# CrystalSixone/VLN-MAGIC

Measured on AMD Instinct MI355X. Metric: trajectory-steps/sec (whole node), MAGIC-S R2R pretrain, higher is better.
Workload: dtype bf16

## Files before the change

include/magic_hip.h:

```cpp
#ifndef MAGIC_HIP_H
#define MAGIC_HIP_H
#ifdef __cplusplus
extern "C" {
#endif

#define MAGIC_OK 0
#define MAGIC_ERR_ARG (-1)
#define MAGIC_ERR_LAUNCH (-2)
#define MAGIC_ERR_UNSUPPORTED (-3)

int magic_abi_version(void);
int magic_build_id(char* out, int len);
int magic_device_info(int* cu_count, int* clock_khz, char* arch, int arch_len);

int magic_gemm(int dtype, int layout, int batch, int nh, int M, int N, int K,
               const void* A, int lda, long long sAb, long long sAh,
               const void* B, int ldb, long long sBb, long long sBh,
               void* C, int ldc, long long sCb, long long sCh, int c_f32, int accumulate,
               const float* bias, int epilogue, const void* aux, int ldaux,
               const void* residual, int ldr, void* C2, int ldc2,
               float alpha, int splitk, float* bias_grad, void* stream);
int magic_gemm_set_big(int mode);
#define MAGIC_GEMM_FORM_PLAIN 0x1
#define MAGIC_GEMM_FORM_XCD 0x2
// ... 209 lines not shown
int magic_sap_fuse_bwd(int B, int K, int Vp, const float* g_raw, const float* l_raw, const float* fuse_raw,
                       const unsigned char* gmask, const unsigned char* lmask, const int* fsrc, const unsigned char* bwmask,
                       int use_gate, const float* dgl, const float* dll, const float* dfl,
                       float* dg_raw, float* dl_raw, float* dfuse_raw, void* stream);

int magic_step_rng(unsigned long long base_seed, unsigned* counter, float rw_temp, int* seed_out, float* rw_out, float* zero_me,
                   float* scale_state, float growth, float backoff, int interval, void* stream);
int magic_seed_scale(const float* scale_dev);
int magic_loss_assemble(const float* rows, int n_rows, const float* row_w, float row_scale, const float* kd_rows, int n_kd,
                        float* slots, const float* rw, float alpha, int has_kd, float* out, void* stream);

int magic_rowgate_fwd(int dtype, int M, int H, int mode, const void* x, const void* e, const float* wx, const float* we,
                      const float* b0, const float* b1, float* out_s, void* out, float* gsave, void* stream);
int magic_rowgate_bwd(int dtype, int M, int H, int mode, const void* x, const void* e, const float* wx, const float* we, const float* gsave,
                      const float* dy, const void* dout, void* dx, void* de, float* dwx, float* dwe, float* db0, float* db1, void* stream);

int magic_sumsq(long long n, const float* g, float* out, void* stream);
int magic_adamw(long long n, float* p, float* g, float* m, float* v, void* shadow, int shadow_dtype,
                float lr, float b1, float b2, float eps, float wd, float step_size,
                const float* sumsq, float max_norm, float gscale, const float* lr_ss, long long n_decay, int zero_grad,
                unsigned* overflow, float* scale_state, int* sched_step, int decay_first, void* stream);
int magic_sumsq_sched(long long n, const float* g, float* out, int* step, float lr0, int warmup, int total, float b1, float b2,
                      float* lr_ss, void* stream);
int magic_sched_step(int* step, float lr0, int warmup, int total, float b1, float b2, float* lr_ss, float* zero_me, void* stream);
int magic_cast(int dtype16, int to16, long long n, const void* x, void* y, void* stream);
int magic_add_n(int dtype, long long n, int count, const void* const* xs, void* y, void* stream);
int magic_add(int dtype, long long n, const void* x, void* y, void* stream);
int magic_dact(int dtype, int kind, long long n, const void* dy, const void* z, void* dz, void* stream);

int magic_view_gather(int dtype, int Np, int V, int D, const void* table, int n_viewpoints, const int* vp_row,
                      const int* order, void* out, void* stream);

int magic_set_f32_mfma(int mode);
int magic_get_f32_mfma(void);

typedef struct {
  const void* Wqkv; const float* bqkv; const void* Wo; const float* bo; const float* g1; const float* be1;
  const void* W1; const float* bi; const void* W2; const float* bo2; const float* g2; const float* be2;
  void *qkv, *P, *Pd, *ctx, *a, *z, *g, *out; float *rstd_a, *rstd_o;
  unsigned site_attn, site_ao, site_out, pad_;
} magic_enc_layer;
typedef struct { const void* x; const unsigned char* kmask; int nsamp, N, ldp, nlayers; magic_enc_layer L[6]; } magic_enc_seg;
typedef struct { magic_enc_seg seg[2]; int nseg; float p_attn, p_hidden, eps, scale; const unsigned* seed;
                 unsigned* sync; int sync_words, pad2_; } magic_enc_params;
int magic_encoder_supported(int dtype, int H, int I, int nh, int N, int nlayers);
int magic_encoder_params_bytes(void);
// ... 72 lines not shown
```

vln-magic_amd/csrc/optim.hip:

```cpp
#include "common.hpp"
#include "group.hpp"

struct SchedArgs { int* step; float lr0; int warmup, total; float b1, b2; float* lr_ss; };
__device__ __forceinline__ void sched_advance(const SchedArgs& a) {
  const int gs = a.step[0];
  a.step[0] = gs + 1;
  const int t = a.step[1] + 1;
  a.step[1] = t;
  double f = gs < a.warmup ? (double)gs / (double)a.warmup : fmax(0.0, (double)(a.total - gs) / (double)(a.total - a.warmup));
  double lr = (double)a.lr0 * f;
  if (lr <= 0.0) lr = 1e-8;
  const double ss = lr * sqrt(1.0 - pow((double)a.b2, (double)t)) / (1.0 - pow((double)a.b1, (double)t));
  a.lr_ss[0] = (float)lr; a.lr_ss[1] = (float)ss;
}
__global__ __launch_bounds__(1024) void sumsq_kernel(long long n, const float* __restrict__ g, float* out, SchedArgs sa) {
  __shared__ float red[16];
  if (sa.step && blockIdx.x == 0 && threadIdx.x == 0) sched_advance(sa);
  float s = 0.f;
  const long long n4 = n >> 2, stride = (long long)gridDim.x * 1024;
  for (long long i = (long long)blockIdx.x * 1024 + threadIdx.x; i < n4; i += 4 * stride) {
    float4 v[4];
#pragma unroll
    for (int u = 0; u < 4; ++u) v[u] = (i + u * stride < n4) ? ((const float4*)g)[i + u * stride] : make_float4(0.f, 0.f, 0.f, 0.f);
#pragma unroll
// ... 26 lines not shown
    if (zero_g)
      for (long long i = (long long)blockIdx.x * 256 + threadIdx.x; i < n; i += (long long)gridDim.x * 256) g[i] = 0.f;
    return;
  }
  if (sumsq && max_norm > 0.f) {
    const float nrm = sqrtf(sumsq[0]) * gscale;
    clip = gscale * fminf(1.f, max_norm / (nrm + 1e-6f));
  }
  for (long long i = (long long)blockIdx.x * 256 + threadIdx.x; i < n; i += (long long)gridDim.x * 256) {
    const float gi = g[i] * clip;
    const float mi = b1 * m[i] + (1.f - b1) * gi;
    const float vi = b2 * v[i] + (1.f - b2) * gi * gi;
    float pi = p[i];
    const bool dec = wd > 0.f && i < n_decay;
    if (dec && decay_first) pi -= lr * wd * pi;
    pi -= step_size * mi / (sqrtf(vi) + eps);
    if (dec && !decay_first) pi -= lr * wd * pi;
    m[i] = mi; v[i] = vi; p[i] = pi;
    if (shadow) shadow[i] = (Hh)pi;
    if (zero_g) g[i] = 0.f;
  }
}

template <typename Hh>
__global__ __launch_bounds__(256) void cast_f32_h16_kernel(long long n, const float* x, Hh* y) {
  const long long n4 = n >> 2;
  for (long long i = (long long)blockIdx.x * 256 + threadIdx.x; i < n4; i += (long long)gridDim.x * 256) {
    const float4 v = ((const float4*)x)[i];
    h16x4<Hh> o; o[0] = (Hh)v.x; o[1] = (Hh)v.y; o[2] = (Hh)v.z; o[3] = (Hh)v.w;
    ((h16x4<Hh>*)y)[i] = o;
  }
  if (blockIdx.x == 0 && threadIdx.x < (n & 3)) y[(n4 << 2) + threadIdx.x] = (Hh)x[(n4 << 2) + threadIdx.x];
}

template <typename Hh>
__global__ __launch_bounds__(256) void cast_h16_f32_kernel(long long n, const Hh* x, float* y) {
  for (long long i = (long long)blockIdx.x * 256 + threadIdx.x; i < n; i += (long long)gridDim.x * 256) y[i] = (float)x[i];
}

template <typename T>
__global__ __launch_bounds__(256) void add_kernel(long long n, const T* x, T* y) {
  for (long long i = (long long)blockIdx.x * 256 + threadIdx.x; i < n; i += (long long)gridDim.x * 256) y[i] = from_f<T>(to_f(y[i]) + to_f(x[i]));
}

struct AddN { const void* x[8]; int n; };
template <typename T>
// ... 34 lines not shown
  return launch_status();
}
extern "C" int magic_sumsq_sched(long long n, const float* g, float* out, int* step, float lr0, int warmup, int total, float b1, float b2,
                                 float* lr_ss, void* stream) {
  if (n <= 0 || ((uintptr_t)g & 15) || !step || !lr_ss || warmup <= 0 || total <= warmup) return MAGIC_ERR_ARG;
  const int nb = nblocks(n, 4096);
  hipLaunchKernelGGL(sumsq_kernel, dim3(nb > 256 ? 256 : nb), dim3(1024), 0, (hipStream_t)stream, n, g, out, SchedArgs{step, lr0, warmup, total, b1, b2, lr_ss});
  return launch_status();
}

extern "C" int magic_adamw(long long n, float* p, float* g, float* m, float* v, void* shadow, int shadow_dtype,
                           float lr, float b1, float b2, float eps, float wd, float step_size,
                           const float* sumsq, float max_norm, float gscale, const float* lr_ss, long long n_decay, int zero_grad,
                           unsigned* overflow, float* scale_state, int* sched_step, int decay_first, void* stream) {
  if (n <= 0 || (shadow && !dtype_is16(shadow_dtype))) return MAGIC_ERR_ARG;
  if (scale_state && !sumsq) return MAGIC_ERR_ARG;
  if (n_decay < 0) n_decay = n;
  if (shadow && shadow_dtype == DT_F16)
    hipLaunchKernelGGL(adamw_kernel<f16>, dim3(nblocks(n, 256)), dim3(256), 0, (hipStream_t)stream, n, p, g, m, v, (f16*)shadow, lr, b1, b2, eps, wd,
                       step_size, sumsq, max_norm, gscale, lr_ss, n_decay, zero_grad, overflow, scale_state, sched_step, decay_first);
  else
    hipLaunchKernelGGL(adamw_kernel<bf16>, dim3(nblocks(n, 256)), dim3(256), 0, (hipStream_t)stream, n, p, g, m, v, (bf16*)shadow, lr, b1, b2, eps, wd,
                       step_size, sumsq, max_norm, gscale, lr_ss, n_decay, zero_grad, overflow, scale_state, sched_step, decay_first);
  return launch_status();
}

extern "C" int magic_cast(int dtype16, int to16, long long n, const void* x, void* y, void* stream) {
  if (n <= 0 || !dtype_is16(dtype16)) return MAGIC_ERR_ARG;
  const hipStream_t st = (hipStream_t)stream;
  if (to16) {
    if (((uintptr_t)x & 15) || ((uintptr_t)y & 7)) return MAGIC_ERR_ARG;
    DISPATCH_H(dtype16, hipLaunchKernelGGL(cast_f32_h16_kernel<TY>, dim3(nblocks(n, 1024)), dim3(256), 0, st, n, (const float*)x, (TY*)y));
  } else {
    DISPATCH_H(dtype16, hipLaunchKernelGGL(cast_h16_f32_kernel<TY>, dim3(nblocks(n, 256)), dim3(256), 0, st, n, (const TY*)x, (float*)y));
  }
  return launch_status();
}

extern "C" int magic_add(int dtype, long long n, const void* x, void* y, void* stream) {
  if (n <= 0) return MAGIC_ERR_ARG;
  DISPATCH_T(dtype, hipLaunchKernelGGL(add_kernel<TY>, dim3(nblocks(n, 256)), dim3(256), 0, (hipStream_t)stream, n, (const TY*)x, (TY*)y));
  return launch_status();
}

extern "C" int magic_add_n(int dtype, long long n, int count, const void* const* xs, void* y, void* stream) {
  if (n <= 0 || count < 1 || count > 8 || !xs || !y || ((uintptr_t)y & 15)) return MAGIC_ERR_ARG;
// ... 109 lines not shown
```

vln-magic_amd/host/ops.py:

```python
import ctypes as C
import os

import torch

from . import lanes
from . import lib as L

FLOPS = {"total": 0.0, "gemm": 0.0, "linear_ln": 0.0, "attn": 0.0, "enc": 0.0, "enabled": False}
BYTES = {"dw": 0.0, "dw_launches": 0}


def _count(m, n, k, batch=1, fam="gemm"):
    if FLOPS["enabled"]:
        f = 2.0 * m * n * k * batch
        FLOPS["total"] += f
        FLOPS[fam] += f


def _chk(cond, msg):
    if not cond:
        raise L.MagicHipError("shape check failed: " + msg)


def gemm(layout, A, B, C, M, N, K, lda, ldb, ldc, *, batch=1, nh=1, sA=(0, 0), sB=(0, 0), sC=(0, 0),
# ... 1268 lines not shown
    _chk(rows.dtype == torch.float32 and rows.is_contiguous() and out.dtype == torch.float32 and out.numel() >= 13, "loss_assemble layout")
    L.call("magic_loss_assemble", L.P(rows), rows.numel(), L.P(row_w), float(row_scale), L.P(kd_rows), kd_rows.numel() if kd_rows is not None else 0,
           L.P(slots), L.P(rw), float(alpha), 1 if has_kd else 0, L.P(out), L.stream())
    return out


def sumsq(g, out):
    L.call("magic_sumsq", g.numel(), L.P(g), L.P(out), L.stream())


def sumsq_sched(g, out, step, lr0, warmup, total, b1, b2, lr_ss):
    _chk(step.numel() >= 2 and step.dtype == torch.int32, "schedule step words: int32[2] {global_step, optimizer state step}")
    L.call("magic_sumsq_sched", g.numel(), L.P(g), L.P(out), L.P(step), float(lr0), int(warmup), int(total), float(b1), float(b2), L.P(lr_ss), L.stream())


def adamw(n, p, g, m, v, shadow, lr, b1, b2, eps, wd, step_size, sumsq_buf, max_norm, gscale, lr_ss=None, n_decay=-1, zero_grad=False, overflow=None,
          scale_state=None, sched_step=None, decay_first=False):
    _chk(sched_step is None or (sched_step.numel() >= 2 and sched_step.dtype == torch.int32), "schedule step words: int32[2] {global_step, optimizer state step}")
    L.call("magic_adamw", n, L.P(p), L.P(g), L.P(m), L.P(v), L.P(shadow), L.dt(shadow.dtype) if shadow is not None else 1, float(lr), float(b1), float(b2), float(eps), float(wd),
           float(step_size), L.P(sumsq_buf), float(max_norm), float(gscale), L.P(lr_ss), int(n_decay), 1 if zero_grad else 0, L.P(overflow),
           L.P(scale_state), L.P(sched_step), 1 if decay_first else 0, L.stream())


def sched_step(step, lr0, warmup, total, b1, b2, lr_ss, zero_me=None):
    _chk(step.numel() >= 2 and step.dtype == torch.int32, "schedule step words: int32[2] {global_step, optimizer state step}")
    L.call("magic_sched_step", L.P(step), float(lr0), int(warmup), int(total), float(b1), float(b2), L.P(lr_ss), L.P(zero_me), L.stream())


def cast_to(x, dtype, out=None):
    if x.dtype == dtype:
        return x
    _chk((x.dtype == torch.float32) != (dtype == torch.float32) and (x.dtype in L.HALF or dtype in L.HALF), "cast_to: fp32 <-> 16-bit only")
    if out is None:
        out = torch.empty(x.shape, dtype=dtype, device=x.device)
    to16 = dtype in L.HALF
    L.call("magic_cast", L.dt(dtype if to16 else x.dtype), 1 if to16 else 0, x.numel(), L.P(x), L.P(out), L.stream())
    return out


def add_(y, x):
    L.call("magic_add", L.dt(y.dtype), y.numel(), L.P(x), L.P(y), L.stream())
    return y


def add_n(y, xs):
    import ctypes as C
# ... 12 lines not shown
```

vln-magic_amd/host/trainer.py:

```python
import math
import os

import torch
import torch.distributed as dist

from .lib import capture as _capture
from . import ops as O
from .plan import build_plan


def warmup_linear(step, warmup, total):
    if step < warmup:
        return step / warmup
    return max(0, (total - step) / (total - warmup))


def get_lr_sched(step, lr, warmup, total):
    v = lr * warmup_linear(step, warmup, total)
    return v if v > 0 else 1e-8


class FusedAdamW:

    def __init__(self, store, lr=5e-5, betas=(0.9, 0.98), eps=1e-6, weight_decay=0.01, max_grad_norm=5.0, schedule=None):
        self.store, self.lr, self.betas, self.eps, self.wd, self.max_norm = store, lr, betas, eps, weight_decay, max_grad_norm
        self.ss = torch.zeros(1, dtype=torch.float32, device=store.device)
        self.overflow = torch.zeros(1, dtype=torch.int32, device=store.device)
        self.loss_scale = None
        self.t = 0
        self.schedule = schedule
        if schedule is not None:
            self.step_dev = torch.zeros(2, dtype=torch.int32, device=store.device)
            self.lr_ss = torch.zeros(2, dtype=torch.float32, device=store.device)

    def skipped_steps(self):
        return int(self.overflow.item())

    def grad_norm_report(self):
        if self._last_gscale is None or not (self.max_norm or self.loss_scale is not None):
            return None
        g = self._last_gscale * (float(self.loss_scale[1].item()) if self.loss_scale is not None else 1.0)
        nrm = math.sqrt(max(float(self.ss.item()), 0.0)) * g
        rep = {"grad_norm": float(f"{nrm:.4e}"), "max_grad_norm": self.max_norm}
        if self.max_norm:
            rep["clip_factor"] = float(f"{min(1.0, self.max_norm / (nrm + 1e-6)):.4e}") if math.isfinite(nrm) else 0.0
        return rep

    _last_gscale = None

    def step(self, lr=None, gscale=1.0, ss_zeroed=False, zero_grad=False):
        s = self.store
        lr = self.lr if lr is None else lr
        self.t += 1
        self._last_gscale = float(gscale)
        b1, b2 = self.betas
        lr_ss = None
        use_clip = self.max_norm is not None and self.max_norm > 0
        need_ss = use_clip or self.loss_scale is not None
        fused_sched = self.schedule is not None and need_ss and ss_zeroed
        if fused_sched:
            O.sumsq_sched(s.grad, self.ss, self.step_dev, self.lr, self.schedule[0], self.schedule[1], b1, b2, self.lr_ss)
            lr_ss, step_size = self.lr_ss, 0.0
        elif self.schedule is not None:
            O.sched_step(self.step_dev, self.lr, self.schedule[0], self.schedule[1], b1, b2, self.lr_ss, zero_me=self.ss if need_ss else None)
            lr_ss, step_size = self.lr_ss, 0.0
        else:
            step_size = lr * math.sqrt(1.0 - b2 ** self.t) / (1.0 - b1 ** self.t)
            if need_ss:
                self.ss.zero_()
        if need_ss and not fused_sched:
            O.sumsq(s.grad, self.ss)
        shadow = s.shadow if s.half else None
        O.adamw(s.total, s.flat, s.grad, s.m, s.v, shadow, lr, b1, b2, self.eps, self.wd, step_size, self.ss if need_ss else None,
                self.max_norm if use_clip else 0.0, gscale, lr_ss=lr_ss, n_decay=s.n_decay, zero_grad=zero_grad, overflow=self.overflow,
                scale_state=self.loss_scale, sched_step=self.step_dev if self.schedule is not None else None)
        s.shadow_clean = True
        if shadow is not None and s.t_spans:
            s.sync_shadow_t(force=True)
        if shadow is not None and s.f_spans:
            s.sync_shadow_f(force=True)
        return lr


class FlatTorchAdamW:

    def __init__(self, store, lr=1e-3, betas=(0.9, 0.999), eps=1e-8, weight_decay=0.01):
        self.store, self.lr, self.betas, self.eps, self.wd = store, lr, betas, eps, weight_decay
        self.ss = torch.zeros(1, dtype=torch.float32, device=store.device)
        self.overflow = torch.zeros(1, dtype=torch.int32, device=store.device)
        self.t = 0

    def zero_grad(self, set_to_none=True):
        if self.t == 0 or not self._clean:
            self.store.zero_grad()
        self._clean = False

    _clean = False

# ... 65 lines not shown
        self.store = store
        self.world = dist.get_world_size() if dist.is_available() and dist.is_initialized() else 1
        self.force = self.world == 1 and bool(os.environ.get("MAGIC_DP_STRUCTURE")) and dist.is_available() and dist.is_initialized()
        self.chunk = chunk_elems
        self.card_shared = self._ranks_share_a_card()
        self.stream = None
        if (self.world > 1 or self.force) and store.device.type == "cuda":
            from . import lanes
            self.stream = lanes.beside([torch.cuda.current_stream(store.device)], device=store.device)
        self.overlap = (not os.environ.get("MAGIC_DDP_NO_OVERLAP")) if overlap is None else overlap
        self.rccl = None
        if self.stream is not None:
            from . import rccl as _rccl
            self.rccl = _rccl.make(store.device)
        g0d, g0n = store.first_offset(LATE_PREFIXES, True), store.first_offset(LATE_PREFIXES, False)
        nd, tot = store.n_decay, store.total
        first, rest = [(g0d, nd), (g0n, tot)], [(0, g0d), (nd, g0n)]
        mid = store.ranges_of(mid_prefixes(store)) if mid_prefixes(store) else []
        mid = [(max(a, lo), min(b, hi)) for a, b in mid for lo, hi in rest if max(a, lo) < min(b, hi)]
        self.buckets = [first, mid, _subtract(rest, mid)]
        self.table = store.offsets.get(EMB_TABLE)
        self.sparse_cap = sparse_rows_cap
        self._pending = []

    def _ranks_share_a_card(self):
        dev = self.store.device
        if self.world == 1 or dev.type != "cuda":
            return False
        import hashlib
        import socket
        props = torch.cuda.get_device_properties(dev)
        me = repr((socket.gethostname(), str(getattr(props, "uuid", "")), getattr(props, "pci_domain_id", -1), getattr(props, "pci_bus_id", -1),
                   getattr(props, "pci_device_id", -1), os.environ.get("HIP_VISIBLE_DEVICES", os.environ.get("CUDA_VISIBLE_DEVICES", "")), dev.index))
        mine = torch.tensor([int.from_bytes(hashlib.sha1(me.encode()).digest()[:7], "big")], dtype=torch.int64, device=dev)
        seen = [torch.zeros_like(mine) for _ in range(self.world)]
        dist.all_gather(seen, mine)
        shared = len({int(t) for t in seen}) < self.world
        if shared:
            O.card_is_shared(True)
        return shared

    def _ranges(self, ranges):
        g = self.store.grad
        if self.rccl is not None:
            with self.rccl.group():
                for lo, hi in ranges:
# ... 19 lines not shown
    def _sparse_rows(self, row_ids, cap=None):
        off, n, (R, H) = self.table
        tab = self.store.grad[off:off + n].view(R, H)
        cap = self.sparse_cap if cap is None else int(cap)
        ids = torch.zeros(cap, dtype=torch.int64, device=tab.device)
        k = int(row_ids.numel())
        if k > cap:
            raise ValueError(f"sparse embedding exchange: {k} touched rows > cap {cap}")
        ids[:k] = row_ids
        rows = tab.index_select(0, ids)
        rows[k:] = 0
        all_ids = torch.empty(self.world * cap, dtype=torch.int64, device=tab.device)
        all_rows = torch.empty(self.world * cap, H, dtype=tab.dtype, device=tab.device)
        if self.rccl is not None:
            with self.rccl.group():
                self.rccl.all_gather(all_ids, ids)
                self.rccl.all_gather(all_rows.view(-1), rows.view(-1))
        else:
            dist.all_gather_into_tensor(all_ids, ids)
            dist.all_gather_into_tensor(all_rows, rows)
        tab.index_fill_(0, row_ids, 0)
        for r in range(self.world):
            tab.index_add_(0, all_ids[r * cap:(r + 1) * cap], all_rows[r * cap:(r + 1) * cap])

    def _sparse_rows_padded(self, ids_pad):
        off, n, (R, H) = self.table
        tab = self.store.grad[off:off + n].view(R, H)
        cap = int(ids_pad.numel())
        valid = ids_pad >= 0
        idx = ids_pad.clamp_min(0)
        rows = tab.index_select(0, idx) * valid.to(tab.dtype)[:, None]
        all_ids = torch.empty(self.world * cap, dtype=torch.int64, device=tab.device)
        all_rows = torch.empty(self.world * cap, H, dtype=tab.dtype, device=tab.device)
        if self.rccl is not None:
            with self.rccl.group():
                self.rccl.all_gather(all_ids, idx)
                self.rccl.all_gather(all_rows.view(-1), rows.view(-1))
        else:
            dist.all_gather_into_tensor(all_ids, idx)
            dist.all_gather_into_tensor(all_rows, rows)
        tab.index_fill_(0, idx, 0)
        for r in range(self.world):
            tab.index_add_(0, all_ids[r * cap:(r + 1) * cap], all_rows[r * cap:(r + 1) * cap])

    def reduce_bucket(self, i, touched_rows=None, cap_scale=1, padded=False):
        if self.world == 1 and not self.force:
            return
        ranges = self.buckets[i]
        last = len(self.buckets) - 1
        sparse = i == last and touched_rows is not None and (padded or touched_rows.numel() > 0) and self.table is not None and self.sparse_cap
        if sparse:
            off, n, _ = self.table
            assert off == 0 and ranges[0][0] == 0
            ranges = [(n, ranges[0][1])] + ranges[1:]

        def run():
            self._ranges(ranges)
            if sparse and padded:
                self._sparse_rows_padded(touched_rows)
            elif sparse:
                self._sparse_rows(touched_rows, cap=self.sparse_cap * cap_scale)
        self._on_side(run)

    def all_reduce(self):
        if self.world == 1 and not self.force:
            return 1.0
        self._on_side(lambda: self._ranges([(0, self.store.total)]))
        self.join()
        return 1.0 / self.world

    def finish(self):
        self.join()
        return 1.0 / self.world if self.world > 1 else 1.0
# ... 191 lines not shown

    def _fwd_bwd_ahead(self, cur, t_cur, nxt, rw=None):
        st = self.student
        self._one_update_per_call("step_ahead / capture_ahead")
        main = torch.cuda.current_stream()
        self.side.wait_stream(main)
        with torch.cuda.stream(self.side):
            t_next = self.teacher_forward(*nxt)
        batch, task, plan = cur
        drawn = self.mkrw()
        if rw is None:
            rw = drawn
        self._zero_grad()
        self._window_rows = [self._touched_rows(task, plan)]
        out = st(batch, task, compute_loss=True, teacher_outputs=t_cur, rw=rw, plan=plan, inputs=t_cur["inputs"])
        hook = self._bucket_hook(task, plan) if not torch.cuda.is_current_stream_capturing() else None
        st.backward(on_bucket=hook)
        self._exchanged = hook is not None
        main.wait_stream(self.side)
        return out, t_next

    def step_ahead(self, cur, t_cur, nxt, rw=None):
        out, t_next = self._fwd_bwd_ahead(cur, t_cur, nxt, rw)
        self._optimize()
        self.global_step += 1
        return out, t_next

    def capture_ahead(self, cur, t_cur, nxt, rw=None, t_next_into=None):
        full = self.sync.world == 1 and not self.sync.force and not os.environ.get("MAGIC_FORCE_SPLIT_GRAPH")
        for b in (cur[0], nxt[0]):
            off = [k for k, v in b.items() if torch.is_tensor(v) and v.device.type != self.dev.type and k not in ("traj_vp_row", "traj_view_order")]
            if off:
                raise ValueError(f"capture_ahead() needs both batches resident on {self.dev}; host tensors: {off[:4]}...")
        g = torch.cuda.CUDAGraph()
        with self._graph_ctx(g):
            out, t_next = self._fwd_bwd_ahead(cur, t_cur, nxt, rw)
            if t_next_into is not None:
                copy_teacher_outputs(t_next, t_next_into)
                t_next = t_next_into
            if full:
                self._optimize()
        cs = CapturedStep(g, out, cur[2]["traj_steps"], full, keep=(cur, t_cur, nxt, rw))
        cs.t_next = t_next
        return cs

    def capture_student(self, cur, t_cur, rw=None, keep=None, rccl_in_graph=True, touched_static=None):
        self._one_update_per_call("capture_student / capture_split")
        full = self.sync.world == 1 and not self.sync.force and not os.environ.get("MAGIC_FORCE_SPLIT_GRAPH")
        batch, task, plan = cur
        two = (not full) and self.sync.overlap and not os.environ.get("MAGIC_DDP_ONE_GRAPH")
        if two and rccl_in_graph and os.environ.get("MAGIC_DDP_GRAPH_RCCL", "1") != "0" and self.sync.stream is not None and self.sync.rccl is not None and self.sync.rccl.graph_ok:
            gS = torch.cuda.CUDAGraph()
            padded = touched_static is not None and task != "mlm" and bool(self.sync.sparse_cap)
            touched = touched_static if padded else self._touched_rows(task, plan)
            with self._graph_ctx(gS):
                drawn = self.mkrw()
                rw_ = drawn if rw is None else rw
                self._zero_grad()
                out = self.student(batch, task, compute_loss=True, teacher_outputs=t_cur, rw=rw_, plan=plan, inputs=t_cur["inputs"])
                self.student.backward(on_bucket=lambda i, ctx: self.sync.reduce_bucket(i, touched if i == 2 else None, padded=padded))
                self._opt_step(self.sync.finish())
            cs = CapturedStep(gS, out, plan["traj_steps"], True, keep=keep if keep is not None else (cur, t_cur, rw, touched))
            cs.graph2 = cs.graph3 = cs.graph_opt = None
            cs.touched, cs.rccl_in_graph = touched, True
            return cs
        gS = torch.cuda.CUDAGraph()
        gS2 = None
        with self._graph_ctx(gS):
            drawn = self.mkrw()
            rw_ = drawn if rw is None else rw
            self._zero_grad()
            out = self.student(batch, task, compute_loss=True, teacher_outputs=t_cur, rw=rw_, plan=plan, inputs=t_cur["inputs"])
            if two:
                self.student.backward_phase1()
                O.flush_dw(keep_active=True)
            else:
                self.student.backward()
            if full:
                self._optimize()
        gS3 = None
        if two:
            gS2, gS3 = torch.cuda.CUDAGraph(), torch.cuda.CUDAGraph()
            state = {"ctx": _capture(gS2, pool=gS.pool(), capture_error_mode="relaxed")}
            state["ctx"].__enter__()

            def cut():
                O.flush_dw(keep_active=True)
                state["ctx"].__exit__(None, None, None)
                state["ctx"] = _capture(gS3, pool=gS.pool(), capture_error_mode="relaxed")
                state["ctx"].__enter__()
            try:
                self.student.backward_phase2(on_cut=cut)
            finally:
                state["ctx"].__exit__(None, None, None)
        cs = CapturedStep(gS, out, plan["traj_steps"], full, keep=keep if keep is not None else (cur, t_cur, rw))
        cs.graph2, cs.graph3, cs.touched = gS2, gS3, self._touched_rows(task, plan)
        cs.graph_opt = None
        if two:
            cs.graph_opt = torch.cuda.CUDAGraph()
            with _capture(cs.graph_opt, pool=gS.pool(), capture_error_mode="relaxed"):
                self._opt_step(1.0 / self.sync.world if self.sync.world > 1 else 1.0)
        return cs

    def replay_student(self, cs, touched=None, between=None):
        O.dw_guard()
        if getattr(cs, "rccl_in_graph", False) and touched is not None and touched is not cs.touched:
            raise ValueError("this step was captured with its bucket collectives (and its touched word-embedding rows) inside the graph: capture it with "
                             "rccl_in_graph=False to pass per-replay row ids")
        cs.graph.replay()
        if getattr(cs, "graph2", None) is not None:
            self.sync.reduce_bucket(0)
            cs.graph2.replay()
            self.sync.reduce_bucket(1)
            cs.graph3.replay()
            self.sync.reduce_bucket(2, touched if touched is not None else cs.touched)
            self._exchanged = True
        if between is not None:
            between()
        if not cs.full:
            if getattr(cs, "graph_opt", None) is not None and self._exchanged:
                self.sync.finish()
                self._exchanged = False
                cs.graph_opt.replay()
                self.opt.t += 1
            else:
                self._optimize()
        self.global_step += 1
        return cs.out

    def capture_split(self, cur, t_cur, nxt, rw=None, t_next_into=None):
        cs = self.capture_student(cur, t_cur, rw=rw, keep=(cur, t_cur, nxt, rw))
        gT = torch.cuda.CUDAGraph()
        with _capture(gT, stream=self.side, capture_error_mode="relaxed"):
            if self.student.will_fuse_encoders(cur[2]):
                O.encoder_start_gate(self.gate)
            t_next = self.teacher_forward(*nxt)
            if t_next_into is not None:
                copy_teacher_outputs(t_next, t_next_into)
                t_next = t_next_into
        cs.t_graph, cs.t_next = gT, t_next
        return cs

    def replay_split(self, cs):
        main = torch.cuda.current_stream()
        if getattr(self, "_t_done", None) is not None:
            main.wait_event(self._t_done)
        self.side.wait_stream(main)

        def teacher_next():
            with torch.cuda.stream(self.side):
                cs.t_graph.replay()
                self._t_done = torch.cuda.Event()
                self._t_done.record(self.side)
        return self.replay_student(cs, between=teacher_next)

    def _optimize(self):
        if getattr(self, "_exchanged", False):
            gscale = self.sync.finish()
            self._exchanged = False
        else:
            gscale = self.sync.all_reduce()
        self._opt_step(gscale)

    def _opt_step(self, gscale):
        static = 1.0 if self.opt.loss_scale is not None else float(getattr(self.student, "grad_scale", 1.0))
        self.opt.step(gscale=gscale / (static * self.accum_steps),
                      ss_zeroed=self._ss_zeroed, zero_grad=True)
        self._ss_zeroed, self._grad_clean = False, True

    def step(self, batch, task, rw=None, plan=None):
        plan = plan if plan is not None else build_plan(batch, task, self.dev)
        out = self._fwd_bwd(batch, task, rw, plan)
        if self._micro == self.accum_steps - 1:
            self._optimize()
            self.global_step += 1
            self._micro = 0
        else:
            self._micro += 1
        return out

    def capture(self, batch, task, plan, rw=None):
        off = [k for k, v in batch.items() if torch.is_tensor(v) and v.device.type != self.dev.type and k not in ("traj_vp_row", "traj_view_order")]
        if off:
            raise ValueError(f"capture() needs the batch resident on {self.dev} (synth.batch_to); host tensors: {off[:4]}...")
        full = self.sync.world == 1 and not self.sync.force and not os.environ.get("MAGIC_FORCE_SPLIT_GRAPH")
        if self.accum_steps != 1:
            raise NotImplementedError("captured steps run one optimizer step per replay: use step() with accum_steps > 1")
        g = torch.cuda.CUDAGraph()
        with self._graph_ctx(g):
            out = self._fwd_bwd(batch, task, rw, plan)
            if full:
                self._optimize()
        return CapturedStep(g, out, plan["traj_steps"], full, keep=(batch, plan, rw))

    def replay(self, cs):
        O.dw_guard()
        cs.graph.replay()
        if not cs.full:
            self._optimize()
        self.global_step += 1
        return cs.out
```

Measured before the change: 197,500.

## Skip untouched embedding-table rows in grad-norm and AdamW update

Adds row-sparse gradient-norm and AdamW kernels. The norm pass reads only the embedding-table rows listed in the touched-id set and marks them in a bitmap. The update kernel uses that bitmap to skip gradient reads and zero-writes for untouched rows, while still updating p/m/v for every row. The trainer now threads touched-row ids through the optimizer paths, including the multi-rank sparse reduce. The aim is to cut gradient memory traffic on a large vocab table, at the cost of atomics, extra host plumbing and more complex kernels.

```diff
diff --git a/include/magic_hip.h b/include/magic_hip.h
--- a/include/magic_hip.h
+++ b/include/magic_hip.h
@@ -255,6 +255,13 @@
                 unsigned* overflow, float* scale_state, int* sched_step, int decay_first, void* stream);
 int magic_sumsq_sched(long long n, const float* g, float* out, int* step, float lr0, int warmup, int total, float b1, float b2,
                       float* lr_ss, void* stream);
+int magic_sumsq_rows(long long n, const float* g, float* out, long long tab_off, int R, int H, const long long* ids, long long nids,
+                     unsigned* bitmap, int* step, float lr0, int warmup, int total, float b1, float b2, float* lr_ss, void* stream);
+int magic_adamw_rows(long long n, float* p, float* g, float* m, float* v, void* shadow, int shadow_dtype,
+                     float lr, float b1, float b2, float eps, float wd, float step_size,
+                     const float* sumsq, float max_norm, float gscale, const float* lr_ss, long long n_decay, int zero_grad,
+                     unsigned* overflow, float* scale_state, int* sched_step, int decay_first,
+                     long long tab_off, int R, int H, unsigned* bitmap, void* stream);
 int magic_sched_step(int* step, float lr0, int warmup, int total, float b1, float b2, float* lr_ss, float* zero_me, void* stream);
 int magic_cast(int dtype16, int to16, long long n, const void* x, void* y, void* stream);
 int magic_add_n(int dtype, long long n, int count, const void* const* xs, void* y, void* stream);
diff --git a/profiles/micro/opt_rows_probe.py b/profiles/micro/opt_rows_probe.py
--- /dev/null
+++ b/profiles/micro/opt_rows_probe.py
@@ -0,0 +1,87 @@
+import os
+import statistics
+import sys
+
+import torch
+
+sys.path.insert(0, os.path.join(os.path.dirname(os.path.abspath(__file__)), "..", ".."))
+import magic_amd
+from magic_amd.host import ops as O
+
+ROUNDS = int(sys.argv[1]) if len(sys.argv) > 1 else 12
+REPS = int(sys.argv[2]) if len(sys.argv) > 2 else 20
+N, R, H = 10_160_000, 50_265, 128
+COPY_ROOF = 6.29e12
+dev = "cuda"
+table = (0, R, H)
+p = torch.randn(N, device=dev)
+g = torch.zeros(N, device=dev)
+m, v = torch.zeros(N, device=dev), torch.zeros(N, device=dev)
+shadow = p.to(torch.bfloat16)
+ss = torch.zeros(1, device=dev)
+step = torch.zeros(2, dtype=torch.int32, device=dev)
+lr_ss = torch.zeros(2, device=dev)
+bitmap = torch.zeros((R + 31) // 32, dtype=torch.int32, device=dev)
+SCHED = (step, 5e-5, 10000, 200000, 0.9, 0.98, lr_ss)
+HYP = (5e-5, 0.9, 0.98, 1e-6, 0.01, 0.0)
+
+
+def refill(ids):
+    ss.zero_()
+    bitmap.zero_()
+    g[R * H:].fill_(1e-3)
+    if ids.numel():
+        g[:R * H].view(R, H).index_fill_(0, ids, 1e-3)
+
+
+def dense(ids, what):
+    if what != "adamw":
+        O.sumsq_sched(g, ss, *SCHED)
+    if what != "sumsq":
+        O.adamw(N, p, g, m, v, shadow, *HYP, ss, 5.0, 1.0, lr_ss=lr_ss, n_decay=N - 4096, zero_grad=True, sched_step=step)
+
+
+def rows(ids, what):
+    O.sumsq_rows(g, ss, table, ids, bitmap, sched=SCHED)
+    if what != "sumsq":
+        O.adamw_rows(N, p, g, m, v, shadow, *HYP, ss, 5.0, 1.0, table, bitmap, lr_ss=lr_ss, n_decay=N - 4096, zero_grad=True, sched_step=step)
+
+
+def timed(fn, ids, what):
+    ev = []
+    for _ in range(REPS):
+        refill(ids)
+        e0, e1 = torch.cuda.Event(enable_timing=True), torch.cuda.Event(enable_timing=True)
+        e0.record()
+        fn(ids, what)
+        e1.record()
+        ev.append((e0, e1))
+    torch.cuda.synchronize()
+    return sum(a.elapsed_time(b) for a, b in ev) * 1e3 / REPS
+
+
+print(f"n = {N}, table {R} x {H} at offset 0, bf16 shadow, zero_grad; {ROUNDS} rounds x {REPS} launches per form, interleaved; us per call (one event pair around each call)")
+print("'both' = norm + update; 'norm' = the norm launch alone; the update alone = both - norm (the rows update needs the norm launch's bitmap)")
+for k in (0, 2400, 3840, R):
+    ids = torch.randperm(R, device=dev)[:k].to(torch.int64).contiguous()
+    for _ in range(3):
+        refill(ids); dense(ids, "both"); refill(ids); rows(ids, "both")
+    torch.cuda.synchronize()
+    t = {key: [] for key in (("dense", "both"), ("rows", "both"), ("dense", "sumsq"), ("rows", "sumsq"))}
+    for r in range(ROUNDS):
+        for (form, what) in t:
+            t[(form, what)].append(timed(dense if form == "dense" else rows, ids, what))
+    torch.cuda.synchronize()
+    refill(ids); rows(ids, "both")
+    torch.cuda.synchronize()
+    assert int(bitmap.count_nonzero()) == 0 and int(g.count_nonzero()) == 0
+    live = N - R * H + k * H
+    b = {("dense", "sumsq"): 4 * N, ("rows", "sumsq"): 4 * live, ("dense", "both"): 38 * N, ("rows", "both"): 38 * live + 26 * (R - k) * H}
+    print(f"\nid list of {k} rows")
+    for key in t:
+        med, mn = statistics.median(t[key]), min(t[key])
+        print(f"  {key[0]:5s} {'norm' if key[1] == 'sumsq' else 'both':4s}  median {med:7.2f} us  min {mn:7.2f} us   {b[key] / 1e6:6.1f} MB moved: {b[key] / med / 1e6:5.2f} TB/s at the median "
+              f"= {100 * b[key] / med / 1e-6 / COPY_ROOF:5.1f} % of the {COPY_ROOF / 1e12:.2f} TB/s float4-copy roof")
+    md = {key: statistics.median(t[key]) for key in t}
+    print(f"  update alone (both - norm): dense {md[('dense', 'both')] - md[('dense', 'sumsq')]:.2f} us, rows {md[('rows', 'both')] - md[('rows', 'sumsq')]:.2f} us")
+    print(f"  difference of medians, both launches: {md[('dense', 'both')] - md[('rows', 'both')]:.2f} us per step; norm alone: {md[('dense', 'sumsq')] - md[('rows', 'sumsq')]:.2f} us")
diff --git a/vln-magic_amd/csrc/optim.hip b/vln-magic_amd/csrc/optim.hip
--- a/vln-magic_amd/csrc/optim.hip
+++ b/vln-magic_amd/csrc/optim.hip
@@ -72,6 +72,160 @@
   }
 }
 
+struct RowTable { long long off; int R, H; };
+
+__global__ __launch_bounds__(1024) void sumsq_rows_kernel(long long n, const float* __restrict__ g, float* out, RowTable tb,
+                                                          const long long* __restrict__ ids, long long nids, unsigned* bitmap, SchedArgs sa) {
+  __shared__ float red[16];
+  if (sa.step && blockIdx.x == 0 && threadIdx.x == 0) sched_advance(sa);
+  const int lane = threadIdx.x & 63;
+  const long long W = (long long)gridDim.x * 16, w = (long long)blockIdx.x * 16 + (threadIdx.x >> 6);
+  auto claim = [&](long long base, long long& id) -> bool {
+    const long long k = base + (long long)lane * W + w;
+    id = k < nids ? ids[k] : -1;
+    if (id < 0 || id >= tb.R) return false;
+    const unsigned bit = 1u << (id & 31);
+    return (atomicOr(bitmap + (id >> 5), bit) & bit) == 0u;
+  };
+  long long id0;
+  const bool mine0 = claim(0, id0);
+  float s = 0.f;
+  const long long h4 = tb.off >> 2, hole4 = ((long long)tb.R * tb.H) >> 2;
+  const long long n4 = (n >> 2) - hole4, stride = (long long)gridDim.x * 1024;
+  for (long long i = (long long)blockIdx.x * 1024 + threadIdx.x; i < n4; i += 4 * stride) {
+    float4 v[4];
+#pragma unroll
+    for (int u = 0; u < 4; ++u) {
+      const long long j = i + u * stride;
+      v[u] = (j < n4) ? ((const float4*)g)[j < h4 ? j : j + hole4] : make_float4(0.f, 0.f, 0.f, 0.f);
+    }
+#pragma unroll
+    for (int u = 0; u < 4; ++u) s += v[u].x * v[u].x + v[u].y * v[u].y + v[u].z * v[u].z + v[u].w * v[u].w;
+  }
+  if (blockIdx.x == 0 && threadIdx.x < (n & 3)) { const float v = g[((n >> 2) << 2) + threadIdx.x]; s += v * v; }
+  const float4* tab = (const float4*)(g + tb.off);
+  const int row4 = tb.H >> 2;
+  for (long long base = 0; base < nids; base += 64 * W) {
+    long long id = id0;
+    const bool mine = base == 0 ? mine0 : claim(base, id);
+    unsigned long long todo = __ballot(mine);
+    while (todo) {
+      const int u = __ffsll((long long)todo) - 1;
+      todo &= todo - 1;
+      const long long r = __shfl(id, u);
+      if (lane < row4) { const float4 x = tab[r * row4 + lane]; s += x.x * x.x + x.y * x.y + x.z * x.z + x.w * x.w; }
+    }
+  }
+  s = wave_sum(s);
+  if (lane == 0) red[threadIdx.x >> 6] = s;
+  __syncthreads();
+  if (threadIdx.x == 0) {
+    float t = 0.f;
+    for (int k = 0; k < 16; ++k) t += red[k];
+    atomicAdd(out, t);
+  }
+}
+
+struct AdamK { float lr, b1, b2, eps, wd, step_size, clip; long long n_decay; int decay_first, zero_g; };
+__device__ __forceinline__ float adamw_elem(const AdamK& k, long long i, float graw, float& m, float& v, float p) {
+  const float gi = __fmul_rn(graw, k.clip);
+  const float mi = __fmaf_rn(k.b1, m, __fmul_rn(1.f - k.b1, gi));
+  const float vi = __fmaf_rn(k.b2, v, __fmul_rn(__fmul_rn(1.f - k.b2, gi), gi));
+  float pi = p;
+  const bool dec = k.wd > 0.f && i < k.n_decay;
+  const float lw = __fmul_rn(k.lr, k.wd);
+  if (dec && k.decay_first) pi = __fmaf_rn(-lw, pi, pi);
+  pi = __fsub_rn(pi, __fdiv_rn(__fmul_rn(k.step_size, mi), __fadd_rn(sqrtf(vi), k.eps)));
+  if (dec && !k.decay_first) pi = __fmaf_rn(-lw, pi, pi);
+  m = mi; v = vi;
+  return pi;
+}
+template <typename Hh>
+__global__ __launch_bounds__(64) void adamw_rows_kernel(long long n, float* p, float* g, float* m, float* v, Hh* shadow,
+                                                         float lr, float b1, float b2, float eps, float wd, float step_size,
+                                                         const float* sumsq, float max_norm, float gscale, const float* lr_ss, long long n_decay, int zero_g,
+                                                         unsigned* overflow, float* scale_state, int* sched_step, int decay_first,
+                                                         RowTable tb, unsigned* bitmap) {
+  if (lr_ss) { lr = lr_ss[0]; step_size = lr_ss[1]; }
+  if (scale_state) gscale *= scale_state[1];
+  const bool bad = sumsq && !isfinite(sumsq[0]);
+  if (scale_state && blockIdx.x == 0 && threadIdx.x == 0) scale_state[3] = bad ? 2.f : 1.f;
+  float clip = gscale;
+  if (bad) {
+    if (sched_step && blockIdx.x == 0 && threadIdx.x == 0) sched_step[1] -= 1;
+    if (overflow && blockIdx.x == 0 && threadIdx.x == 0) atomicAdd(overflow, 1u);
+  } else if (sumsq && max_norm > 0.f) {
+    const float nrm = sqrtf(sumsq[0]) * gscale;
+    clip = gscale * fminf(1.f, max_norm / (nrm + 1e-6f));
+  }
+  const AdamK k = {lr, b1, b2, eps, wd, step_size, clip, n_decay, decay_first, zero_g};
+  const int lane = threadIdx.x;
+  const int words = (tb.R + 31) >> 5, lg4 = tb.H == 128 ? 5 : 6;
+  const long long h4 = tb.off >> 2, hole4 = ((long long)tb.R * tb.H) >> 2, o4 = (n >> 2) - hole4;
+  const long long tasks = words + ((o4 + 1023) >> 10);
+  const float4 zero4 = make_float4(0.f, 0.f, 0.f, 0.f);
+  for (long long t = blockIdx.x; t < tasks; t += gridDim.x) {
+    long long q0; int c4, sh; unsigned word;
+    if (t < words) {
+      const int r0 = (int)t << 5, nr = tb.R - r0 < 32 ? tb.R - r0 : 32;
+      word = bitmap[t]; q0 = h4 + ((long long)r0 << lg4); c4 = nr << lg4; sh = lg4;
+    } else {
+      const long long a = (t - words) << 10;
+      word = 1u; q0 = a; c4 = (int)(o4 - a < 1024 ? o4 - a : 1024); sh = 10;
+    }
+    const bool in_table = t < words;
+    const int trips = (c4 + 255) >> 8, first = (int)(t % trips);
+    for (int trip = 0; trip < trips; ++trip) {
+      const int j0 = (((first + trip) % trips) << 8) + lane;
+      long long q[4]; bool live[4], hg[4];
+#pragma unroll
+      for (int u = 0; u < 4; ++u) {
+        const int j = j0 + 64 * u;
+        live[u] = j < c4;
+        const long long l = q0 + (live[u] ? j : 0);
+        q[u] = in_table ? l : (l < h4 ? l : l + hole4);
+        hg[u] = live[u] && ((word >> (j >> sh)) & 1u);
+      }
+      if (bad) {
+#pragma unroll
+        for (int u = 0; u < 4; ++u)
+          if (zero_g && hg[u]) ((float4*)g)[q[u]] = zero4;
+        continue;
+      }
+      float4 P[4], G[4], M[4], V[4];
+#pragma unroll
+      for (int u = 0; u < 4; ++u) { P[u] = ((const float4*)p)[q[u]]; M[u] = ((const float4*)m)[q[u]]; V[u] = ((const float4*)v)[q[u]]; }
+#pragma unroll
+      for (int u = 0; u < 4; ++u) G[u] = hg[u] ? ((const float4*)g)[q[u]] : zero4;
+#pragma unroll
+      for (int u = 0; u < 4; ++u) {
+        if (!live[u]) continue;
+        const long long i = q[u] << 2;
+        P[u].x = adamw_elem(k, i, G[u].x, M[u].x, V[u].x, P[u].x);
+        P[u].y = adamw_elem(k, i + 1, G[u].y, M[u].y, V[u].y, P[u].y);
+        P[u].z = adamw_elem(k, i + 2, G[u].z, M[u].z, V[u].z, P[u].z);
+        P[u].w = adamw_elem(k, i + 3, G[u].w, M[u].w, V[u].w, P[u].w);
+        ((float4*)m)[q[u]] = M[u]; ((float4*)v)[q[u]] = V[u]; ((float4*)p)[q[u]] = P[u];
+        if (shadow) {
+          h16x4<Hh> o; o[0] = (Hh)P[u].x; o[1] = (Hh)P[u].y; o[2] = (Hh)P[u].z; o[3] = (Hh)P[u].w;
+          ((h16x4<Hh>*)shadow)[q[u]] = o;
+        }
+        if (zero_g && hg[u]) ((float4*)g)[q[u]] = zero4;
+      }
+    }
+    if (in_table && word && lane == 0) bitmap[t] = 0u;
+  }
+  if (blockIdx.x == 0 && threadIdx.x < (n & 3)) {
+    const long long i = ((n >> 2) << 2) + threadIdx.x;
+    if (bad) { if (zero_g) g[i] = 0.f; return; }
+    float mi = m[i], vi = v[i];
+    const float pi = adamw_elem(k, i, g[i], mi, vi, p[i]);
+    m[i] = mi; v[i] = vi; p[i] = pi;
+    if (shadow) shadow[i] = (Hh)pi;
+    if (zero_g) g[i] = 0.f;
+  }
+}
+
 template <typename Hh>
 __global__ __launch_bounds__(256) void cast_f32_h16_kernel(long long n, const float* x, Hh* y) {
   const long long n4 = n >> 2;
@@ -152,6 +306,41 @@
   else
     hipLaunchKernelGGL(adamw_kernel<bf16>, dim3(nblocks(n, 256)), dim3(256), 0, (hipStream_t)stream, n, p, g, m, v, (bf16*)shadow, lr, b1, b2, eps, wd,
                        step_size, sumsq, max_norm, gscale, lr_ss, n_decay, zero_grad, overflow, scale_state, sched_step, decay_first);
+  return launch_status();
+}
+
+static inline bool row_table_ok(long long n, long long off, int R, int H, const unsigned* bitmap) {
+  return bitmap && !((uintptr_t)bitmap & 3) && R > 0 && (H == 128 || H == 256) && off >= 0 && !(off & 3) && off + (long long)R * H <= n;
+}
+
+extern "C" int magic_sumsq_rows(long long n, const float* g, float* out, long long tab_off, int R, int H, const long long* ids, long long nids,
+                                unsigned* bitmap, int* step, float lr0, int warmup, int total, float b1, float b2, float* lr_ss, void* stream) {
+  if (n <= 0 || ((uintptr_t)g & 15) || !row_table_ok(n, tab_off, R, H, bitmap) || nids < 0 || (nids > 0 && (!ids || ((uintptr_t)ids & 7)))) return MAGIC_ERR_ARG;
+  if (step && (!lr_ss || warmup <= 0 || total <= warmup)) return MAGIC_ERR_ARG;
+  const int nb = nblocks(n, 4096);
+  hipLaunchKernelGGL(sumsq_rows_kernel, dim3(nb > 256 ? 256 : nb), dim3(1024), 0, (hipStream_t)stream, n, g, out, RowTable{tab_off, R, H}, ids, nids, bitmap,
+                     step ? SchedArgs{step, lr0, warmup, total, b1, b2, lr_ss} : SchedArgs{});
+  return launch_status();
+}
+
+extern "C" int magic_adamw_rows(long long n, float* p, float* g, float* m, float* v, void* shadow, int shadow_dtype,
+                                float lr, float b1, float b2, float eps, float wd, float step_size,
+                                const float* sumsq, float max_norm, float gscale, const float* lr_ss, long long n_decay, int zero_grad,
+                                unsigned* overflow, float* scale_state, int* sched_step, int decay_first,
+                                long long tab_off, int R, int H, unsigned* bitmap, void* stream) {
+  if (n <= 0 || (shadow && !dtype_is16(shadow_dtype))) return MAGIC_ERR_ARG;
+  if (scale_state && !sumsq) return MAGIC_ERR_ARG;
+  if (!row_table_ok(n, tab_off, R, H, bitmap) || (((uintptr_t)p | (uintptr_t)g | (uintptr_t)m | (uintptr_t)v) & 15) || ((uintptr_t)shadow & 7)) return MAGIC_ERR_ARG;
+  if (n_decay < 0) n_decay = n;
+  const RowTable tb = {tab_off, R, H};
+  const long long tasks = ((R + 31) >> 5) + ((((n >> 2) - (((long long)R * H) >> 2)) + 1023) >> 10);
+  const int nb = (int)(tasks > 65536 ? 65536 : tasks);
+  if (shadow && shadow_dtype == DT_F16)
+    hipLaunchKernelGGL(adamw_rows_kernel<f16>, dim3(nb), dim3(64), 0, (hipStream_t)stream, n, p, g, m, v, (f16*)shadow, lr, b1, b2, eps, wd,
+                       step_size, sumsq, max_norm, gscale, lr_ss, n_decay, zero_grad, overflow, scale_state, sched_step, decay_first, tb, bitmap);
+  else
+    hipLaunchKernelGGL(adamw_rows_kernel<bf16>, dim3(nb), dim3(64), 0, (hipStream_t)stream, n, p, g, m, v, (bf16*)shadow, lr, b1, b2, eps, wd,
+                       step_size, sumsq, max_norm, gscale, lr_ss, n_decay, zero_grad, overflow, scale_state, sched_step, decay_first, tb, bitmap);
   return launch_status();
 }
 
diff --git a/vln-magic_amd/host/ops.py b/vln-magic_amd/host/ops.py
--- a/vln-magic_amd/host/ops.py
+++ b/vln-magic_amd/host/ops.py
@@ -1314,6 +1314,29 @@
            L.P(scale_state), L.P(sched_step), 1 if decay_first else 0, L.stream())
 
 
+def rows_table_ok(n, off, R, H):
+    return R > 0 and H in (128, 256) and off >= 0 and off % 4 == 0 and off + R * H <= n
+
+
+def sumsq_rows(g, out, table, ids, bitmap, sched=None):
+    off, R, H = table
+    _chk(ids.dtype == torch.int64 and ids.is_contiguous() and bitmap.dtype == torch.int32 and bitmap.numel() >= (R + 31) // 32, "sumsq_rows: int64 ids, int32 bitmap of ceil(rows / 32) words")
+    step, lr0, warmup, total, b1, b2, lr_ss = sched if sched is not None else (None, 0.0, 0, 0, 0.0, 0.0, None)
+    _chk(step is None or (step.numel() >= 2 and step.dtype == torch.int32), "schedule step words: int32[2] {global_step, optimizer state step}")
+    L.call("magic_sumsq_rows", g.numel(), L.P(g), L.P(out), int(off), int(R), int(H), L.P(ids) if ids.numel() else None, ids.numel(), L.P(bitmap),
+           L.P(step), float(lr0), int(warmup), int(total), float(b1), float(b2), L.P(lr_ss), L.stream())
+
+
+def adamw_rows(n, p, g, m, v, shadow, lr, b1, b2, eps, wd, step_size, sumsq_buf, max_norm, gscale, table, bitmap, lr_ss=None, n_decay=-1, zero_grad=False,
+               overflow=None, scale_state=None, sched_step=None, decay_first=False):
+    off, R, H = table
+    _chk(sched_step is None or (sched_step.numel() >= 2 and sched_step.dtype == torch.int32), "schedule step words: int32[2] {global_step, optimizer state step}")
+    _chk(bitmap.dtype == torch.int32 and bitmap.numel() >= (R + 31) // 32, "adamw_rows: int32 bitmap of ceil(rows / 32) words")
+    L.call("magic_adamw_rows", n, L.P(p), L.P(g), L.P(m), L.P(v), L.P(shadow), L.dt(shadow.dtype) if shadow is not None else 1, float(lr), float(b1), float(b2), float(eps),
+           float(wd), float(step_size), L.P(sumsq_buf), float(max_norm), float(gscale), L.P(lr_ss), int(n_decay), 1 if zero_grad else 0, L.P(overflow),
+           L.P(scale_state), L.P(sched_step), 1 if decay_first else 0, int(off), int(R), int(H), L.P(bitmap), L.stream())
+
+
 def sched_step(step, lr0, warmup, total, b1, b2, lr_ss, zero_me=None):
     _chk(step.numel() >= 2 and step.dtype == torch.int32, "schedule step words: int32[2] {global_step, optimizer state step}")
     L.call("magic_sched_step", L.P(step), float(lr0), int(warmup), int(total), float(b1), float(b2), L.P(lr_ss), L.P(zero_me), L.stream())
diff --git a/vln-magic_amd/host/trainer.py b/vln-magic_amd/host/trainer.py
--- a/vln-magic_amd/host/trainer.py
+++ b/vln-magic_amd/host/trainer.py
@@ -29,6 +29,11 @@
         self.loss_scale = None
         self.t = 0
         self.schedule = schedule
+        self.rows_table = self.rows_bitmap = None
+        tab = store.offsets.get(EMB_TABLE) if os.environ.get("MAGIC_OPT_ROWS", "0") != "0" else None
+        if tab is not None and len(tab[2]) == 2 and O.rows_table_ok(store.total, tab[0], tab[2][0], tab[2][1]):
+            self.rows_table = (tab[0], tab[2][0], tab[2][1])
+            self.rows_bitmap = torch.zeros((tab[2][0] + 31) // 32, dtype=torch.int32, device=store.device)
         if schedule is not None:
             self.step_dev = torch.zeros(2, dtype=torch.int32, device=store.device)
             self.lr_ss = torch.zeros(2, dtype=torch.float32, device=store.device)
@@ -48,7 +53,7 @@
 
     _last_gscale = None
 
-    def step(self, lr=None, gscale=1.0, ss_zeroed=False, zero_grad=False):
+    def step(self, lr=None, gscale=1.0, ss_zeroed=False, zero_grad=False, touched_rows=None):
         s = self.store
         lr = self.lr if lr is None else lr
         self.t += 1
@@ -58,8 +63,13 @@
         use_clip = self.max_norm is not None and self.max_norm > 0
         need_ss = use_clip or self.loss_scale is not None
         fused_sched = self.schedule is not None and need_ss and ss_zeroed
+        rows = touched_rows if (touched_rows is not None and need_ss and self.rows_table is not None) else None
         if fused_sched:
-            O.sumsq_sched(s.grad, self.ss, self.step_dev, self.lr, self.schedule[0], self.schedule[1], b1, b2, self.lr_ss)
+            sched = (self.step_dev, self.lr, self.schedule[0], self.schedule[1], b1, b2, self.lr_ss)
+            if rows is not None:
+                O.sumsq_rows(s.grad, self.ss, self.rows_table, rows, self.rows_bitmap, sched=sched)
+            else:
+                O.sumsq_sched(s.grad, self.ss, *sched)
             lr_ss, step_size = self.lr_ss, 0.0
         elif self.schedule is not None:
             O.sched_step(self.step_dev, self.lr, self.schedule[0], self.schedule[1], b1, b2, self.lr_ss, zero_me=self.ss if need_ss else None)
@@ -69,11 +79,19 @@
             if need_ss:
                 self.ss.zero_()
         if need_ss and not fused_sched:
-            O.sumsq(s.grad, self.ss)
+            if rows is not None:
+                O.sumsq_rows(s.grad, self.ss, self.rows_table, rows, self.rows_bitmap)
+            else:
+                O.sumsq(s.grad, self.ss)
         shadow = s.shadow if s.half else None
-        O.adamw(s.total, s.flat, s.grad, s.m, s.v, shadow, lr, b1, b2, self.eps, self.wd, step_size, self.ss if need_ss else None,
-                self.max_norm if use_clip else 0.0, gscale, lr_ss=lr_ss, n_decay=s.n_decay, zero_grad=zero_grad, overflow=self.overflow,
-                scale_state=self.loss_scale, sched_step=self.step_dev if self.schedule is not None else None)
+        kw = dict(lr_ss=lr_ss, n_decay=s.n_decay, zero_grad=zero_grad, overflow=self.overflow, scale_state=self.loss_scale,
+                  sched_step=self.step_dev if self.schedule is not None else None)
+        if rows is not None:
+            O.adamw_rows(s.total, s.flat, s.grad, s.m, s.v, shadow, lr, b1, b2, self.eps, self.wd, step_size, self.ss, self.max_norm if use_clip else 0.0,
+                         gscale, self.rows_table, self.rows_bitmap, **kw)
+        else:
+            O.adamw(s.total, s.flat, s.grad, s.m, s.v, shadow, lr, b1, b2, self.eps, self.wd, step_size, self.ss if need_ss else None,
+                    self.max_norm if use_clip else 0.0, gscale, **kw)
         s.shadow_clean = True
         if shadow is not None and s.t_spans:
             s.sync_shadow_t(force=True)
@@ -185,6 +203,7 @@
         self.table = store.offsets.get(EMB_TABLE)
         self.sparse_cap = sparse_rows_cap
         self._pending = []
+        self.table_ids = None
 
     def _ranks_share_a_card(self):
         dev = self.store.device
@@ -250,6 +269,7 @@
         tab.index_fill_(0, row_ids, 0)
         for r in range(self.world):
             tab.index_add_(0, all_ids[r * cap:(r + 1) * cap], all_rows[r * cap:(r + 1) * cap])
+        self.table_ids = all_ids
 
     def _sparse_rows_padded(self, ids_pad):
         off, n, (R, H) = self.table
@@ -270,6 +290,12 @@
         tab.index_fill_(0, idx, 0)
         for r in range(self.world):
             tab.index_add_(0, all_ids[r * cap:(r + 1) * cap], all_rows[r * cap:(r + 1) * cap])
+        self.table_ids = all_ids
+
+    def table_rows(self, own):
+        if self.world == 1 and not self.force:
+            return own
+        return self.table_ids
 
     def reduce_bucket(self, i, touched_rows=None, cap_scale=1, padded=False):
         if self.world == 1 and not self.force:
@@ -277,6 +303,8 @@
         ranges = self.buckets[i]
         last = len(self.buckets) - 1
         sparse = i == last and touched_rows is not None and (padded or touched_rows.numel() > 0) and self.table is not None and self.sparse_cap
+        if i == last:
+            self.table_ids = None
         if sparse:
             off, n, _ = self.table
             assert off == 0 and ranges[0][0] == 0
@@ -514,7 +542,7 @@
 
     def step_ahead(self, cur, t_cur, nxt, rw=None):
         out, t_next = self._fwd_bwd_ahead(cur, t_cur, nxt, rw)
-        self._optimize()
+        self._optimize_rows(self._window_touched())
         self.global_step += 1
         return out, t_next
 
@@ -531,7 +559,7 @@
                 copy_teacher_outputs(t_next, t_next_into)
                 t_next = t_next_into
             if full:
-                self._optimize()
+                self._optimize_rows(self._window_touched())
         cs = CapturedStep(g, out, cur[2]["traj_steps"], full, keep=(cur, t_cur, nxt, rw))
         cs.t_next = t_next
         return cs
@@ -551,7 +579,8 @@
                 self._zero_grad()
                 out = self.student(batch, task, compute_loss=True, teacher_outputs=t_cur, rw=rw_, plan=plan, inputs=t_cur["inputs"])
                 self.student.backward(on_bucket=lambda i, ctx: self.sync.reduce_bucket(i, touched if i == 2 else None, padded=padded))
-                self._opt_step(self.sync.finish())
+                gscale = self.sync.finish()
+                self._opt_step(gscale, self.sync.table_rows(touched))
             cs = CapturedStep(gS, out, plan["traj_steps"], True, keep=keep if keep is not None else (cur, t_cur, rw, touched))
             cs.graph2 = cs.graph3 = cs.graph_opt = None
             cs.touched, cs.rccl_in_graph = touched, True
@@ -569,7 +598,7 @@
             else:
                 self.student.backward()
             if full:
-                self._optimize()
+                self._optimize_rows(self._touched_rows(task, plan))
         gS3 = None
         if two:
             gS2, gS3 = torch.cuda.CUDAGraph(), torch.cuda.CUDAGraph()
@@ -616,7 +645,7 @@
                 cs.graph_opt.replay()
                 self.opt.t += 1
             else:
-                self._optimize()
+                self._optimize_rows(touched if touched is not None else cs.touched)
         self.global_step += 1
         return cs.out
 
@@ -646,25 +675,35 @@
                 self._t_done.record(self.side)
         return self.replay_student(cs, between=teacher_next)
 
+    def _optimize_rows(self, touched):
+        self._own_rows = touched
+        self._optimize()
+
+    _own_rows = None
+
     def _optimize(self):
+        touched, self._own_rows = self._own_rows, None
         if getattr(self, "_exchanged", False):
             gscale = self.sync.finish()
             self._exchanged = False
+            touched = self.sync.table_rows(touched)
         else:
             gscale = self.sync.all_reduce()
-        self._opt_step(gscale)
-
-    def _opt_step(self, gscale):
+            if self.sync.world > 1 or self.sync.force:
+                touched = None
+        self._opt_step(gscale, touched)
+
+    def _opt_step(self, gscale, touched=None):
         static = 1.0 if self.opt.loss_scale is not None else float(getattr(self.student, "grad_scale", 1.0))
         self.opt.step(gscale=gscale / (static * self.accum_steps),
-                      ss_zeroed=self._ss_zeroed, zero_grad=True)
+                      ss_zeroed=self._ss_zeroed, zero_grad=True, touched_rows=touched)
         self._ss_zeroed, self._grad_clean = False, True
 
     def step(self, batch, task, rw=None, plan=None):
         plan = plan if plan is not None else build_plan(batch, task, self.dev)
         out = self._fwd_bwd(batch, task, rw, plan)
         if self._micro == self.accum_steps - 1:
-            self._optimize()
+            self._optimize_rows(self._window_touched())
             self.global_step += 1
             self._micro = 0
         else:
@@ -681,14 +720,17 @@
         g = torch.cuda.CUDAGraph()
         with self._graph_ctx(g):
             out = self._fwd_bwd(batch, task, rw, plan)
+            touched = self._window_touched()
             if full:
-                self._optimize()
-        return CapturedStep(g, out, plan["traj_steps"], full, keep=(batch, plan, rw))
+                self._optimize_rows(touched)
+        cs = CapturedStep(g, out, plan["traj_steps"], full, keep=(batch, plan, rw, touched))
+        cs.touched = touched
+        return cs
 
     def replay(self, cs):
         O.dw_guard()
         cs.graph.replay()
         if not cs.full:
-            self._optimize()
+            self._optimize_rows(getattr(cs, "touched", None))
         self.global_step += 1
         return cs.out
```

Result: no change. 197,500 (-0.0%).
